# papuSpartan/stable-diffusion-webui-distributed

Hardware: NVIDIA H100
Metric: images/sec SD1.5 512x512 txt2img (higher is better)
Workload: dtype fp16

## Files before the change

stable-diffusion-webui-distributed_b200/b200sd/csrc/gemm_conv_tc.cu:

```cuda
#include <math.h>
#include <stddef.h>
#include <stdlib.h>
#include "tc_common.cuh"
#include "wgmma.cuh"
#include "b200sd_internal.h"
#include "pdl.cuh"

namespace b200sd {

constexpr int kBlockM = 128;
constexpr int kBlockK = 64;
constexpr int kMmaK = 16;
constexpr int kConsumerThreads = 256;
constexpr int kGemmThreads = kConsumerThreads + 128;
constexpr int kMaxStages = 8;
constexpr int kChunkCols = 32;
constexpr uint32_t kStageTileBytes = kBlockM * kChunkCols * 2;
constexpr uint32_t kATileBytes = kBlockM * kBlockK * 2;

struct GemmKernelParams {
  int M, N, K;
  int block_n;
  int num_m_tiles, num_n_tiles, num_k_blocks, num_stages;
  uint32_t a_bytes, b_bytes, d_bytes;
  int mode;
  int H, W, NB;
  int bw, bh, bn;
  int tiles_x, tiles_y;
  int taps, cblocks, stride, pad;
  const float* bias;
  int bias_group_rows;
  int has_residual;
  int flags;
  float res_scale;
};

struct __align__(8) GemmBarriers {
  uint64_t full[kMaxStages];
  uint64_t empty[kMaxStages];
  uint64_t res_full[2];
};

__device__ __forceinline__ float rcp_approx(float x) {
  float y;
  asm("rcp.approx.ftz.f32 %0, %1;" : "=f"(y) : "f"(x));
  return y;
}
__device__ __forceinline__ float gelu_erf(float x) {
  const float z = __fmul_rn(fabsf(x), 0.70710678118654752440f);
  float q = __fmaf_rn(0.0000430638f, z, 0.0002765672f);
  q = __fmaf_rn(q, z, 0.0001520143f);
  q = __fmaf_rn(q, z, 0.0092705272f);
  q = __fmaf_rn(q, z, 0.0422820123f);
  q = __fmaf_rn(q, z, 0.0705230784f);
  q = __fmaf_rn(q, z, 1.0f);
  q = __fmul_rn(q, q);
  q = __fmul_rn(q, q);
  q = __fmul_rn(q, q);
  q = __fmul_rn(q, q);
  const float h = __fmaf_rn(0.5f, copysignf(1.0f - rcp_approx(q), x), 0.5f);
  return __fmul_rn(x, h);
}

template <bool kBf16>
__device__ __forceinline__ uint32_t pack2(float a, float b) {
  if constexpr (kBf16) {
    __nv_bfloat162 v = __floats2bfloat162_rn(a, b);
    return *reinterpret_cast<uint32_t*>(&v);
  } else {
    __half2 v = __floats2half2_rn(a, b);
    return *reinterpret_cast<uint32_t*>(&v);
  }
}
template <bool kBf16>
__device__ __forceinline__ float2 unpack2(uint32_t u) {
  if constexpr (kBf16) {
    return __bfloat1622float2(*reinterpret_cast<__nv_bfloat162*>(&u));
  } else {
    return __half22float2(*reinterpret_cast<__half2*>(&u));
  }
}

__device__ __forceinline__ void consumer_bar_sync() {
  asm volatile("bar.sync 1, %0;" ::"n"(kConsumerThreads) : "memory");
}

struct TileCoord {
  int c1, c2, c3;
};

__device__ __forceinline__ TileCoord tile_coord(const GemmKernelParams& p, int m_tile) {
  TileCoord t;
  if (p.mode == 0) {
    t.c1 = m_tile * kBlockM; t.c2 = 0; t.c3 = 0;
  } else {
    t.c1 = (m_tile % p.tiles_x) * p.bw;
    t.c2 = ((m_tile / p.tiles_x) % p.tiles_y) * p.bh;
    t.c3 = (m_tile / (p.tiles_x * p.tiles_y)) * p.bn;
  }
  return t;
}

__device__ __forceinline__ long long tile_row(const GemmKernelParams& p, const TileCoord& tc, int m_tile, int r) {
  if (p.mode == 0) {
    const long long row = static_cast<long long>(m_tile) * kBlockM + r;
    return row < p.M ? row : 0;
  }
  const int x = tc.c1 + r % p.bw, y = tc.c2 + (r / p.bw) % p.bh, n = tc.c3 + r / (p.bw * p.bh);
  return (x < p.W && y < p.H && n < p.NB && r < p.bw * p.bh * p.bn) ? (static_cast<long long>(n) * p.H + y) * p.W + x : 0;
}

__device__ __forceinline__ void load_residual(const GemmKernelParams& p, const CUtensorMap* tmR, GemmBarriers* bars,
                                              uint8_t* stage_r, const TileCoord& tc, int n_tile, int out_bn, int c) {
  const int buf = c & 1;
  mbar_arrive_expect_tx(&bars->res_full[buf], p.d_bytes);
  const int col = n_tile * out_bn + c * kChunkCols;
  uint8_t* dst = stage_r + buf * kStageTileBytes;
  if (p.mode == 0) tma_load_2d(dst, tmR, &bars->res_full[buf], col, tc.c1);
  else tma_load_4d(dst, tmR, &bars->res_full[buf], col, tc.c1, tc.c2, tc.c3);
}

template <int BN, bool kBf16, bool kScaled>
__device__ __forceinline__ void gemm_conv_tc_body(const CUtensorMap& tmA, const CUtensorMap& tmB,
                                                  const CUtensorMap& tmD, const CUtensorMap& tmR,
                                                  const GemmKernelParams p) {
  constexpr uint32_t kStageBytes = kATileBytes + BN * 128u;
  extern __shared__ uint8_t smem_raw[];
  uint8_t* smem = reinterpret_cast<uint8_t*>((reinterpret_cast<uintptr_t>(smem_raw) + 1023) & ~uintptr_t(1023));
  uint8_t* stage_d = smem + static_cast<size_t>(p.num_stages) * kStageBytes;
  uint8_t* stage_r = stage_d + 2 * kStageTileBytes;
  GemmBarriers* bars = reinterpret_cast<GemmBarriers*>(stage_r + (p.has_residual ? 2 * kStageTileBytes : 0));

  pdl_trigger();
  const int warp = threadIdx.x >> 5;
  const int lane = threadIdx.x & 31;
  const int num_items = p.num_m_tiles * p.num_n_tiles;

  if (threadIdx.x == kConsumerThreads) {
    tma_prefetch_desc(&tmA);
    tma_prefetch_desc(&tmB);
    tma_prefetch_desc(&tmD);
    if (p.has_residual) tma_prefetch_desc(&tmR);
    for (int s = 0; s < p.num_stages; ++s) {
      mbar_init(&bars->full[s], 1);
      mbar_init(&bars->empty[s], kConsumerThreads / 128);
    }
    mbar_init(&bars->res_full[0], 1);
    mbar_init(&bars->res_full[1], 1);
    fence_mbar_init();
  }
  __syncthreads();
  pdl_wait();

  if (warp >= kConsumerThreads / 32) {
    producer_warpgroup_regs();
    if (threadIdx.x == kConsumerThreads) {
      const int nkb = p.num_k_blocks, nstages = p.num_stages, cblocks = p.cblocks;
      const bool conv = p.mode == 1, taps9 = p.taps == 9;
      const uint32_t tx_bytes = p.a_bytes + p.b_bytes;
      int stage = 0;
      uint32_t phase = 0;
      for (int item = blockIdx.x; item < num_items; item += gridDim.x) {
        const int n_tile = item % p.num_n_tiles;
        const int m_tile = item / p.num_n_tiles;
        int cx = 0, cy = 0, cn = 0;
        if (conv) {
          const int tx = m_tile % p.tiles_x;
          const int ty = (m_tile / p.tiles_x) % p.tiles_y;
          cn = (m_tile / (p.tiles_x * p.tiles_y)) * p.bn;
          cx = tx * p.bw * p.stride - p.pad;
          cy = ty * p.bh * p.stride - p.pad;
        }
        const int b_row = n_tile * BN;
        const int a_row = m_tile * kBlockM;
        int cb = 0, dx = 0, dy = 0;
        for (int kb = 0; kb < nkb; ++kb) {
          mbar_wait(&bars->empty[stage], phase ^ 1u);
          uint8_t* sA = smem + static_cast<size_t>(stage) * kStageBytes;
          uint8_t* sB = sA + kATileBytes;
          uint64_t* full_bar = &bars->full[stage];
          mbar_arrive_expect_tx(full_bar, tx_bytes);
          if (!conv) tma_load_2d(sA, &tmA, full_bar, kb * kBlockK, a_row);
          else tma_load_4d(sA, &tmA, full_bar, cb * kBlockK, cx + dx, cy + dy, cn);
          tma_load_2d(sB, &tmB, full_bar, kb * kBlockK, b_row);
          if (++cb == cblocks) {
            cb = 0;
            if (taps9 && ++dx == 3) { dx = 0; ++dy; }
          }
          if (++stage == nstages) { stage = 0; phase ^= 1u; }
        }
      }
    }
    return;
  }

  consumer_warpgroup_regs();
  const int wg = warp >> 2;
  const int row0 = wg * 64 + (warp & 3) * 16 + (lane >> 2);
  const int colq = (lane & 3) * 2;
  const bool signaller = (threadIdx.x & 127) == 0;
  const bool leader = threadIdx.x == 0;
  const bool geglu = (p.flags & B200SD_EPI_GEGLU) != 0;
  const int out_bn = geglu ? BN / 2 : BN;
  const int nchunks = out_bn / kChunkCols;
  const uint32_t smem0 = smem_u32(smem);
  float acc[BN / 2];
  int stage = 0;
  uint32_t phase = 0;
  uint32_t res_uses[2] = {0u, 0u};
  uint32_t d_slot = 0;

  for (int item = blockIdx.x; item < num_items; item += gridDim.x) {
    const int n_tile = item % p.num_n_tiles;
    const int m_tile = item / p.num_n_tiles;
    const TileCoord tc = tile_coord(p, m_tile);
    if (p.has_residual && leader) {
      load_residual(p, &tmR, bars, stage_r, tc, n_tile, out_bn, 0);
      if (nchunks > 1) load_residual(p, &tmR, bars, stage_r, tc, n_tile, out_bn, 1);
    }

    int prev_stage = 0;
    for (int kb = 0; kb < p.num_k_blocks; ++kb) {
      mbar_wait(&bars->full[stage], phase);
      const uint32_t a_addr = smem0 + static_cast<uint32_t>(stage) * kStageBytes + static_cast<uint32_t>(wg) * 8192u;
      const uint32_t b_addr = smem0 + static_cast<uint32_t>(stage) * kStageBytes + kATileBytes;
      reg_fence(acc);
      wgmma_fence();
#pragma unroll
      for (int k = 0; k < kBlockK / kMmaK; ++k)
        Wgmma<BN, kBf16>::ss(acc, make_gdesc_sw128(a_addr + 32u * k, 16, 1024), make_gdesc_sw128(b_addr + 32u * k, 16, 1024),
                             (kb | k) != 0 ? 1u : 0u);
      wgmma_commit();
      reg_fence(acc);
      wgmma_wait<1>();
      if (kb > 0 && signaller) mbar_arrive(&bars->empty[prev_stage]);
      prev_stage = stage;
      if (++stage == p.num_stages) { stage = 0; phase ^= 1u; }
    }
    wgmma_wait<0>();
    reg_fence(acc);
    if (signaller) mbar_arrive(&bars->empty[prev_stage]);

    const float* bias_r[2] = {p.bias, p.bias};
    if (p.bias != nullptr && p.bias_group_rows > 0) {
#pragma unroll
      for (int h = 0; h < 2; ++h) bias_r[h] = p.bias + (tile_row(p, tc, m_tile, row0 + 8 * h) / p.bias_group_rows) * p.N;
    }
#pragma unroll
    for (int c = 0; c < BN / kChunkCols; ++c) {
      if (c < nchunks) {
        float f[2][4][2];
#pragma unroll
        for (int g = 0; g < 4; ++g) {
          const int col = n_tile * BN + c * kChunkCols + g * 8 + colq;
#pragma unroll
          for (int h = 0; h < 2; ++h) {
            float2 b = make_float2(0.f, 0.f), bg = make_float2(0.f, 0.f);
            if (p.bias != nullptr) {
              b = __ldg(reinterpret_cast<const float2*>(bias_r[h] + col));
              if (geglu) bg = __ldg(reinterpret_cast<const float2*>(bias_r[h] + col + BN / 2));
            }
#pragma unroll
            for (int e = 0; e < 2; ++e) {
              const int idx = 4 * (4 * c + g) + 2 * h + e;
              float v = acc[idx] + (e ? b.y : b.x);
              if (geglu) {
                constexpr int kGate = BN / 4;
                v *= gelu_erf(acc[(idx + kGate) % (BN / 2)] + (e ? bg.y : bg.x));
              }
              if constexpr (kScaled) {
                if (p.flags & B200SD_EPI_LRELU) v = v > 0.f ? v : v * 0.2f;
              }
              f[h][g][e] = v;
            }
          }
        }
        if (p.has_residual) {
          const int buf = c & 1;
          mbar_wait(&bars->res_full[buf], res_uses[buf] & 1u);
          res_uses[buf]++;
          const uint8_t* rt = stage_r + buf * kStageTileBytes;
#pragma unroll
          for (int h = 0; h < 2; ++h)
#pragma unroll
            for (int g = 0; g < 4; ++g) {
              const float2 t = unpack2<kBf16>(*reinterpret_cast<const uint32_t*>(rt + sw64_offset(row0 + 8 * h, g) + colq * 2));
              if constexpr (kScaled) {
                f[h][g][0] = __fmaf_rn(p.res_scale, f[h][g][0], t.x);
                f[h][g][1] = __fmaf_rn(p.res_scale, f[h][g][1], t.y);
              } else {
                f[h][g][0] += t.x;
                f[h][g][1] += t.y;
              }
            }
        }
        if (!kScaled && (p.flags & B200SD_EPI_SILU)) {
#pragma unroll
          for (int h = 0; h < 2; ++h)
#pragma unroll
            for (int g = 0; g < 4; ++g)
#pragma unroll
              for (int e = 0; e < 2; ++e) f[h][g][e] = __fdividef(f[h][g][e], 1.0f + __expf(-f[h][g][e]));
        }
        uint8_t* dt = stage_d + d_slot * kStageTileBytes;
#pragma unroll
        for (int h = 0; h < 2; ++h)
#pragma unroll
          for (int g = 0; g < 4; ++g)
            *reinterpret_cast<uint32_t*>(dt + sw64_offset(row0 + 8 * h, g) + colq * 2) = pack2<kBf16>(f[h][g][0], f[h][g][1]);
        fence_proxy_async_smem();
        if (leader) bulk_wait_read<0>();
        consumer_bar_sync();
        if (leader) {
          const int col = n_tile * out_bn + c * kChunkCols;
          if (p.mode == 0) tma_store_2d(&tmD, dt, col, tc.c1);
          else tma_store_4d(&tmD, dt, col, tc.c1, tc.c2, tc.c3);
          bulk_commit();
          if (p.has_residual && c + 2 < nchunks) load_residual(p, &tmR, bars, stage_r, tc, n_tile, out_bn, c + 2);
        }
        d_slot ^= 1u;
      }
    }
  }
  if (leader) bulk_wait<0>();
}

template <int BN, bool kBf16>
__global__ void __launch_bounds__(kGemmThreads, 1)
gemm_conv_tc_kernel(const __grid_constant__ CUtensorMap tmA, const __grid_constant__ CUtensorMap tmB,
                    const __grid_constant__ CUtensorMap tmD, const __grid_constant__ CUtensorMap tmR,
                    const GemmKernelParams p) {
  gemm_conv_tc_body<BN, kBf16, false>(tmA, tmB, tmD, tmR, p);
}

template <int BN, bool kBf16>
__global__ void __launch_bounds__(kGemmThreads, 1)
conv_scaled_tc_kernel(const __grid_constant__ CUtensorMap tmA, const __grid_constant__ CUtensorMap tmB,
                      const __grid_constant__ CUtensorMap tmD, const __grid_constant__ CUtensorMap tmR,
                      const GemmKernelParams p) {
  gemm_conv_tc_body<BN, kBf16, true>(tmA, tmB, tmD, tmR, p);
}

typedef void (*GemmKernel)(CUtensorMap, CUtensorMap, CUtensorMap, CUtensorMap, GemmKernelParams);

static GemmKernel scaled_kernel_for(int block_n, int is_bf16) {
  if (is_bf16) return nullptr;
  if (block_n == 32) return conv_scaled_tc_kernel<32, false>;
  if (block_n == 64) return conv_scaled_tc_kernel<64, false>;
  return nullptr;
}

template <bool kBf16>
static GemmKernel kernel_for(int block_n) {
  switch (block_n) {
    case 32: return gemm_conv_tc_kernel<32, kBf16>;
    case 64: return gemm_conv_tc_kernel<64, kBf16>;
    case 96: return gemm_conv_tc_kernel<96, kBf16>;
    case 128: return gemm_conv_tc_kernel<128, kBf16>;
    case 160: return gemm_conv_tc_kernel<160, kBf16>;
    case 192: return gemm_conv_tc_kernel<192, kBf16>;
    case 224: return gemm_conv_tc_kernel<224, kBf16>;
    case 256: return gemm_conv_tc_kernel<256, kBf16>;
    default: return nullptr;
  }
}
static GemmKernel kernel_for(int block_n, int is_bf16) {
  return is_bf16 ? kernel_for<true>(block_n) : kernel_for<false>(block_n);
}

static int g_num_sms = 0;
static int g_max_smem = 0;
static bool g_dev_ready[64] = {};
static int device_props() {
  int dev = 0;
  if (cudaGetDevice(&dev) != cudaSuccess) return B200SD_ERR_CUDA;
  if (dev < 0 || dev >= 64) return B200SD_ERR_UNSUPPORTED;
  if (!g_dev_ready[dev]) {
    int sms = 0, smem = 0;
    if (cudaDeviceGetAttribute(&sms, cudaDevAttrMultiProcessorCount, dev) != cudaSuccess) return B200SD_ERR_CUDA;
    if (cudaDeviceGetAttribute(&smem, cudaDevAttrMaxSharedMemoryPerBlockOptin, dev) != cudaSuccess)
      return B200SD_ERR_CUDA;
    for (int bn = 32; bn <= 256; bn += 32)
      for (int bf = 0; bf < 2; ++bf)
        for (GemmKernel k : {kernel_for(bn, bf), scaled_kernel_for(bn, bf)})
          if (k != nullptr && cudaFuncSetAttribute(k, cudaFuncAttributeMaxDynamicSharedMemorySize, smem) != cudaSuccess)
            return B200SD_ERR_CUDA;
    g_num_sms = sms;
    g_max_smem = smem;
    g_dev_ready[dev] = true;
  }
  return B200SD_OK;
}

static int launch(const CUtensorMap& tmA, const CUtensorMap& tmB, const CUtensorMap& tmD, const CUtensorMap& tmR,
                  GemmKernelParams& p, int is_bf16, int max_ctas, cudaStream_t stream, bool scaled = false) {
  const uint32_t stage_bytes = kATileBytes + static_cast<uint32_t>(p.block_n) * 128u;
  const int staging = (p.has_residual ? 4 : 2) * static_cast<int>(kStageTileBytes);
  const int budget = g_max_smem - 1024  - staging - static_cast<int>(sizeof(GemmBarriers));
  int stages = budget / static_cast<int>(stage_bytes);
  if (stages > kMaxStages) stages = kMaxStages;
  if (stages < 2) return B200SD_ERR_UNSUPPORTED;
  p.num_stages = stages;
  const size_t smem = 1024 + static_cast<size_t>(stages) * stage_bytes + staging + sizeof(GemmBarriers);
  const int num_tiles = p.num_m_tiles * p.num_n_tiles;
  int grid = num_tiles < g_num_sms ? num_tiles : g_num_sms;
  if (max_ctas > 0 && grid > max_ctas) grid = max_ctas;
  if (grid <= 0) return B200SD_OK;
  GemmKernel k = scaled ? scaled_kernel_for(p.block_n, is_bf16) : kernel_for(p.block_n, is_bf16);
  if (k == nullptr) return B200SD_ERR_INVALID;
  launch_pdl(k, dim3(grid), dim3(kGemmThreads), smem, stream, tmA, tmB, tmD, tmR, p);
  return cudaGetLastError() == cudaSuccess ? B200SD_OK : B200SD_ERR_CUDA;
}

struct OutSpec {
  void* D;
  long long ldd;
  const void* residual;
  long long ldr;
  int n_out;
};

static int fill_common(GemmKernelParams& p, OutSpec& o, int M, int N, int K, int block_n, const b200sd_epilogue* epi,
                       void* D, long long ldd, int is_bf16) {
  if (block_n < 32 || block_n > 256 || block_n % 32 != 0 || N % block_n != 0 || K % kBlockK != 0) return B200SD_ERR_INVALID;
  p.M = M; p.N = N; p.K = K; p.block_n = block_n;
  p.num_n_tiles = N / block_n;
  p.num_k_blocks = K / kBlockK;
  p.b_bytes = static_cast<uint32_t>(block_n) * 128u;
  p.bias = epi ? epi->bias : nullptr;
  p.bias_group_rows = epi ? epi->bias_group_rows : 0;
  p.flags = epi ? epi->flags : 0;
  o.D = D; o.ldd = ldd;
  o.residual = epi ? epi->residual : nullptr;
  o.ldr = epi ? epi->ldr : 0;
  p.has_residual = o.residual != nullptr ? 1 : 0;
  const bool geglu = (p.flags & B200SD_EPI_GEGLU) != 0;
  if (geglu && block_n % 64 != 0) return B200SD_ERR_INVALID;
  o.n_out = geglu ? N / 2 : N;
  if (ldd % 8 != 0 || (reinterpret_cast<uintptr_t>(D) & 15) != 0) return B200SD_ERR_INVALID;
  if (o.residual && (o.ldr % 8 != 0 || (reinterpret_cast<uintptr_t>(o.residual) & 15) != 0)) return B200SD_ERR_INVALID;
  if (p.bias && (reinterpret_cast<uintptr_t>(p.bias) & 15) != 0) return B200SD_ERR_INVALID;
  return B200SD_OK;
}

static int make_out_maps(const GemmKernelParams& p, const OutSpec& o, CUtensorMap* tmD, CUtensorMap* tmR) {
  int rc;
  for (int which = 0; which < 2; ++which) {
    const void* base = which == 0 ? o.D : o.residual;
    const long long ld = which == 0 ? o.ldd : o.ldr;
    CUtensorMap* out = which == 0 ? tmD : tmR;
    if (base == nullptr) {
      *tmR = *tmD;
      continue;
    }
    if (p.mode == 0) {
      const uint64_t dims[2] = {static_cast<uint64_t>(o.n_out), static_cast<uint64_t>(p.M)};
      const uint64_t strides[1] = {static_cast<uint64_t>(ld) * 2};
      const uint32_t box[2] = {kChunkCols, kBlockM};
      const uint32_t es[2] = {1, 1};
      rc = make_tmap_sw64(out, base, 2, dims, strides, box, es);
    } else {
      const uint64_t dims[4] = {static_cast<uint64_t>(o.n_out), static_cast<uint64_t>(p.W), static_cast<uint64_t>(p.H),
                                static_cast<uint64_t>(p.NB)};
      const uint64_t strides[3] = {static_cast<uint64_t>(ld) * 2, static_cast<uint64_t>(ld) * 2 * p.W,
                                   static_cast<uint64_t>(ld) * 2 * p.W * p.H};
      const uint32_t box[4] = {kChunkCols, static_cast<uint32_t>(p.bw), static_cast<uint32_t>(p.bh),
                               static_cast<uint32_t>(p.bn)};
      const uint32_t es[4] = {1, 1, 1, 1};
      rc = make_tmap_sw64(out, base, 4, dims, strides, box, es);
    }
    if (rc != B200SD_OK) return rc;
  }
  return B200SD_OK;
}

int gemm_tc(const void* A, long long lda, const void* Wt, void* D, long long ldd, int M, int N, int K, int block_n,
            const b200sd_epilogue* epi, int is_bf16, int max_ctas, cudaStream_t stream) {
  if (M <= 0) return B200SD_OK;
  GemmKernelParams p{};
  OutSpec o{};
  int rc = fill_common(p, o, M, N, K, block_n, epi, D, ldd, is_bf16);
  if (rc != B200SD_OK) return rc;
  if (lda % 8 != 0 || (reinterpret_cast<uintptr_t>(A) & 15) != 0 || (reinterpret_cast<uintptr_t>(Wt) & 15) != 0)
    return B200SD_ERR_INVALID;
  p.mode = 0;
  p.num_m_tiles = (M + kBlockM - 1) / kBlockM;
  p.a_bytes = 16384u;
  p.d_bytes = kStageTileBytes;
  rc = device_props();
  if (rc != B200SD_OK) return rc;
  CUtensorMap tmA, tmB, tmD, tmR;
  {
    const uint64_t dims[2] = {static_cast<uint64_t>(K), static_cast<uint64_t>(M)};
    const uint64_t strides[1] = {static_cast<uint64_t>(lda) * 2};
    const uint32_t box[2] = {kBlockK, kBlockM};
    const uint32_t es[2] = {1, 1};
    rc = make_tmap_sw128(&tmA, A, 2, dims, strides, box, es);
    if (rc != B200SD_OK) return rc;
  }
  {
    const uint64_t dims[2] = {static_cast<uint64_t>(K), static_cast<uint64_t>(N)};
    const uint64_t strides[1] = {static_cast<uint64_t>(K) * 2};
    const uint32_t box[2] = {kBlockK, static_cast<uint32_t>(block_n)};
    const uint32_t es[2] = {1, 1};
    rc = make_tmap_sw128(&tmB, Wt, 2, dims, strides, box, es);
    if (rc != B200SD_OK) return rc;
  }
  rc = make_out_maps(p, o, &tmD, &tmR);
  if (rc != B200SD_OK) return rc;
  return launch(tmA, tmB, tmD, tmR, p, is_bf16, max_ctas, stream);
}

int conv_tc(const void* X, long long pitch_c, int NB, int Hin, int Win, int C, const void* Wt, int ksize, int stride,
            int pad, int pad_end, void* D, long long ldd, int Cout, int block_n, const b200sd_epilogue* epi,
            int is_bf16, int max_ctas, cudaStream_t stream, bool scaled, float res_scale) {
  if (NB <= 0) return B200SD_OK;
  if ((ksize != 3 && ksize != 1) || (stride != 1 && stride != 2) || C % kBlockK != 0) return B200SD_ERR_INVALID;
  if (scaled && epi != nullptr && (epi->flags & ~B200SD_EPI_LRELU) != 0) return B200SD_ERR_INVALID;
  if (pitch_c % 8 != 0 || (reinterpret_cast<uintptr_t>(X) & 15) != 0 || (reinterpret_cast<uintptr_t>(Wt) & 15) != 0)
    return B200SD_ERR_INVALID;
  const int taps = ksize * ksize;
  const int Ho = (Hin + pad + pad_end - ksize) / stride + 1;
  const int Wo = (Win + pad + pad_end - ksize) / stride + 1;
  if (Ho <= 0 || Wo <= 0) return B200SD_ERR_INVALID;
  GemmKernelParams p{};
  OutSpec o{};
  int rc = fill_common(p, o, NB * Ho * Wo, Cout, taps * C, block_n, epi, D, ldd, is_bf16);
  if (rc != B200SD_OK) return rc;
  p.mode = 1;
  p.res_scale = res_scale;
  p.H = Ho; p.W = Wo; p.NB = NB;
  p.taps = taps; p.cblocks = C / kBlockK; p.stride = stride; p.pad = pad;
  p.bw = Wo < kBlockM ? Wo : kBlockM;
  p.bh = kBlockM / p.bw; if (p.bh > Ho) p.bh = Ho; if (p.bh < 1) p.bh = 1;
  p.bn = kBlockM / (p.bw * p.bh); if (p.bn > NB) p.bn = NB; if (p.bn < 1) p.bn = 1;
  p.tiles_x = (Wo + p.bw - 1) / p.bw;
  p.tiles_y = (Ho + p.bh - 1) / p.bh;
  const int tiles_n = (NB + p.bn - 1) / p.bn;
  p.num_m_tiles = p.tiles_x * p.tiles_y * tiles_n;
  p.a_bytes = static_cast<uint32_t>(p.bw * p.bh * p.bn) * 128u;
  p.d_bytes = static_cast<uint32_t>(p.bw * p.bh * p.bn) * kChunkCols * 2u;
  rc = device_props();
  if (rc != B200SD_OK) return rc;
  CUtensorMap tmA, tmB, tmD, tmR;
  {
    const uint64_t dims[4] = {static_cast<uint64_t>(C), static_cast<uint64_t>(Win), static_cast<uint64_t>(Hin),
                              static_cast<uint64_t>(NB)};
    const uint64_t strides[3] = {static_cast<uint64_t>(pitch_c) * 2, static_cast<uint64_t>(pitch_c) * 2 * Win,
                                 static_cast<uint64_t>(pitch_c) * 2 * Win * Hin};
    const uint32_t box[4] = {kBlockK, static_cast<uint32_t>(p.bw * stride), static_cast<uint32_t>(p.bh * stride),
                             static_cast<uint32_t>(p.bn)};
    const uint32_t es[4] = {1, static_cast<uint32_t>(stride), static_cast<uint32_t>(stride), 1};
    if (box[1] > 256 || box[2] > 256) return B200SD_ERR_UNSUPPORTED;
    rc = make_tmap_sw128(&tmA, X, 4, dims, strides, box, es);
    if (rc != B200SD_OK) return rc;
  }
  {
    const uint64_t K = static_cast<uint64_t>(taps) * C;
    const uint64_t dims[2] = {K, static_cast<uint64_t>(Cout)};
    const uint64_t strides[1] = {K * 2};
    const uint32_t box[2] = {kBlockK, static_cast<uint32_t>(block_n)};
    const uint32_t es[2] = {1, 1};
    rc = make_tmap_sw128(&tmB, Wt, 2, dims, strides, box, es);
    if (rc != B200SD_OK) return rc;
  }
  rc = make_out_maps(p, o, &tmD, &tmR);
  if (rc != B200SD_OK) return rc;
  return launch(tmA, tmB, tmD, tmR, p, is_bf16, max_ctas, stream, scaled);
}

}
```

stable-diffusion-webui-distributed_b200/b200sd/ops.py:

```python
import ctypes
from typing import Optional

import torch

from . import _lib
from ._lib import BF16, EPI_GEGLU, EPI_LRELU, EPI_SILU, F16, Epilogue, check

LAUNCHES = 0


def _count(n: int = 1):
    global LAUNCHES
    LAUNCHES += n


def _dt(t: torch.Tensor) -> int:
    if t.dtype == torch.float16:
        return F16
    if t.dtype == torch.bfloat16:
        return BF16
    raise TypeError(f"b200sd ops take fp16/bf16 activations, got {t.dtype}")


def _stream() -> ctypes.c_void_p:
    return ctypes.c_void_p(torch.cuda.current_stream().cuda_stream)


def _p(t: Optional[torch.Tensor]) -> ctypes.c_void_p:
    return ctypes.c_void_p(0 if t is None else t.data_ptr())


def _rows2d(t: torch.Tensor):
    assert t.stride(-1) == 1, "last dim must be contiguous"
    cols = t.shape[-1]
    pitch = t.stride(-2) if t.dim() >= 2 else cols
    rows = t.numel() // cols
    exp = pitch
    for d in range(t.dim() - 2, -1, -1):
        if t.shape[d] != 1:
            assert t.stride(d) == exp, f"tensor is not row-collapsible: shape {tuple(t.shape)} stride {t.stride()}"
        exp *= t.shape[d]
    return rows, cols, pitch


def _epi(bias, bias_group_rows, residual, flags):
    e = Epilogue()
    e.bias = 0 if bias is None else bias.data_ptr()
    e.bias_group_rows = int(bias_group_rows)
    e.residual = 0 if residual is None else residual.data_ptr()
    e.ldr = 0 if residual is None else _rows2d(residual)[2]
    e.flags = int(flags)
    if bias is not None:
        assert bias.dtype == torch.float32 and bias.is_contiguous()
    return e


NUM_SMS = 132


def pick_block_n(n: int, geglu: bool = False, m: Optional[int] = None) -> int:
    cands = [bn for bn in (160, 128, 96, 64, 32) if n % bn == 0 and (not geglu or bn % 64 == 0)]
    if not cands:
        raise ValueError(f"N={n} has no supported tile width")
    if geglu or m is None:
        return cands[0]
    mt = (m + 127) // 128
    best = None
    for bn in cands:
        if bn < 128 <= cands[0]:
            continue
        tiles = mt * (n // bn)
        waves = -(-tiles // NUM_SMS)
        score = tiles / (waves * NUM_SMS) * (1.0 if bn >= 160 else 0.97 if bn >= 128 else 0.93)
        if best is None or score > best[0] + 1e-9:
            best = (score, bn)
    return best[1]


def linear(a: torch.Tensor, wt: torch.Tensor, out: torch.Tensor, bias: Optional[torch.Tensor] = None,
           bias_group_rows: int = 0, residual: Optional[torch.Tensor] = None, flags: int = 0,
           block_n: Optional[int] = None, max_ctas: int = 0):
    m, k, lda = _rows2d(a)
    n, k2 = wt.shape
    assert k == k2 and wt.is_contiguous()
    mo, no, ldd = _rows2d(out)
    geglu = bool(flags & EPI_GEGLU)
    assert mo == m and no == (n // 2 if geglu else n), (mo, m, no, n)
    bn = block_n or pick_block_n(n, geglu, m)
    e = _epi(bias, bias_group_rows, residual, flags)
    rc = _lib.lib().b200sd_linear(_p(a), ctypes.c_longlong(lda), _p(wt), _p(out), ctypes.c_longlong(ldd), m, n, k, bn,
                                  ctypes.byref(e), _dt(a), max_ctas, _stream())
    check(rc, f"b200sd_linear M={m} N={n} K={k} bn={bn}")
    _count()
    return out


def conv2d(x: torch.Tensor, wt: torch.Tensor, out: torch.Tensor, ksize: int, stride: int = 1, pad: int = 1,
           pad_end: Optional[int] = None, bias: Optional[torch.Tensor] = None, bias_group_rows: int = 0,
           residual: Optional[torch.Tensor] = None, flags: int = 0, block_n: Optional[int] = None, max_ctas: int = 0):
    nb, h, w, c = x.shape
    assert x.stride(3) == 1 and x.stride(1) == w * x.stride(2) and x.stride(0) == h * x.stride(1)
    cout, kk = wt.shape
    assert kk == ksize * ksize * c and wt.is_contiguous()
    pe = pad if pad_end is None else pad_end
    mo, no, ldd = _rows2d(out)
    bn = block_n or pick_block_n(cout, False, mo)
    e = _epi(bias, bias_group_rows, residual, flags)
    rc = _lib.lib().b200sd_conv2d(_p(x), ctypes.c_longlong(x.stride(2)), nb, h, w, c, _p(wt), ksize, stride, pad, pe,
                                  _p(out), ctypes.c_longlong(ldd), cout, bn, ctypes.byref(e), _dt(x), max_ctas,
                                  _stream())
    check(rc, f"b200sd_conv2d NB={nb} H={h} W={w} C={c} Cout={cout} k={ksize} s={stride}")
    _count()
    return out


def attention(q: torch.Tensor, k: torch.Tensor, v: torch.Tensor, out: torch.Tensor, heads: int, d: int, d_pad: int,
              scale: float, v_ones_col: bool = False, kv_len: Optional[torch.Tensor] = None):
    b, sq, _ = q.shape
    skv = k.shape[1]
    for t in (q, k, v, out):
        assert t.stride(2) == 1 and t.stride(0) == t.shape[1] * t.stride(1)
    if kv_len is None:
        rc = _lib.lib().b200sd_attention(_p(q), ctypes.c_longlong(q.stride(1)), _p(k), ctypes.c_longlong(k.stride(1)),
                                         _p(v), ctypes.c_longlong(v.stride(1)), _p(out), ctypes.c_longlong(out.stride(1)),
                                         b, heads, sq, skv, d, d_pad, ctypes.c_float(scale), int(bool(v_ones_col)),
                                         _dt(q), _stream())
        check(rc, f"b200sd_attention B={b} h={heads} Sq={sq} Skv={skv} d={d}")
    else:
        assert kv_len.dtype == torch.int32 and kv_len.is_contiguous() and kv_len.numel() == b
        assert kv_len.device == q.device, "kv_len must live on the device"
        rc = _lib.lib().b200sd_attention_varlen(_p(q), ctypes.c_longlong(q.stride(1)), _p(k),
                                                ctypes.c_longlong(k.stride(1)), _p(v), ctypes.c_longlong(v.stride(1)),
                                                _p(out), ctypes.c_longlong(out.stride(1)), b, heads, sq, skv,
                                                _p(kv_len), d, d_pad, ctypes.c_float(scale), int(bool(v_ones_col)),
                                                _dt(q), _stream())
        check(rc, f"b200sd_attention_varlen B={b} h={heads} Sq={sq} Skv={skv} d={d}")
    _count()
    return out


_GN_FLOATS = {}


def groupnorm_stats_floats(nb: int, hw: int, c: int, groups: int) -> int:
    key = (nb, hw, c, groups)
    n = _GN_FLOATS.get(key)
    if n is None:
        n = int(_lib.lib().b200sd_groupnorm_stats_floats(nb, hw, c, groups))
        if n < 0:
            raise _lib.B200SDError(f"groupnorm: unsupported shape C={c}")
        _GN_FLOATS[key] = n
    return n


def groupnorm(x: torch.Tensor, out: torch.Tensor, stats: torch.Tensor, gamma: torch.Tensor, beta: torch.Tensor,
              groups: int, eps: float, silu: bool):
    nb, hw, c = x.shape
    assert x.stride(2) == 1 and out.stride(2) == 1 and x.stride(0) == hw * x.stride(1)
    assert stats.dtype == torch.float32 and stats.is_contiguous()
    assert stats.numel() >= groupnorm_stats_floats(nb, hw, c, groups), "stats buffer too small"
    rc = _lib.lib().b200sd_groupnorm(_p(x), ctypes.c_longlong(x.stride(1)), _p(out), ctypes.c_longlong(out.stride(1)), nb,
                                     hw, c, groups, _p(stats), _p(gamma), _p(beta), ctypes.c_float(eps), int(silu),
                                     _dt(x), _stream())
    check(rc, "b200sd_groupnorm")
    _count(2)
    return out


def layernorm(x: torch.Tensor, out: torch.Tensor, gamma: torch.Tensor, beta: torch.Tensor, eps: float = 1e-5):
    rows, c, ldx = _rows2d(x)
    _, _, ldy = _rows2d(out)
    rc = _lib.lib().b200sd_layernorm(_p(x), ctypes.c_longlong(ldx), _p(out), ctypes.c_longlong(ldy), rows, c, _p(gamma),
                                     _p(beta), ctypes.c_float(eps), _dt(x), _stream())
    check(rc, "b200sd_layernorm")
    _count()
    return out


def upsample2x(x: torch.Tensor, out: torch.Tensor):
    nb, h, w, c = x.shape
    rc = _lib.lib().b200sd_upsample2x(_p(x), ctypes.c_longlong(x.stride(2)), _p(out), ctypes.c_longlong(out.stride(2)),
                                      nb, h, w, c, _dt(x), _stream())
    check(rc, "b200sd_upsample2x")
    _count()
    return out


def pad_circular(x: torch.Tensor, out: torch.Tensor, p: int):
    nb, h, w, c = x.shape
    for t in (x, out):
        assert t.stride(3) == 1 and t.stride(1) == t.shape[2] * t.stride(2) and t.stride(0) == t.shape[1] * t.stride(1)
    assert out.shape == (nb, h + 2 * p, w + 2 * p, c) and out.dtype == x.dtype, (tuple(x.shape), tuple(out.shape), p)
    rc = _lib.lib().b200sd_pad_circular(_p(x), ctypes.c_longlong(x.stride(2)), _p(out), ctypes.c_longlong(out.stride(2)),
                                        nb, h, w, c, p, _dt(x), _stream())
    check(rc, f"b200sd_pad_circular NB={nb} H={h} W={w} C={c} p={p}")
    _count()
    return out


def softmax_rows_(s: torch.Tensor, scale: float):
    rows, cols, lds = _rows2d(s)
    rc = _lib.lib().b200sd_softmax_rows(_p(s), ctypes.c_longlong(lds), rows, cols, ctypes.c_float(scale), _dt(s),
                                        _stream())
    check(rc, "b200sd_softmax_rows")
    _count()
    return s


def silu(x: torch.Tensor, out: torch.Tensor):
    assert x.is_contiguous() and out.is_contiguous()
    rc = _lib.lib().b200sd_silu(_p(x), _p(out), ctypes.c_longlong(x.numel()), _dt(x), _stream())
    check(rc, "b200sd_silu")
    _count()
    return out


def timestep_embedding(t: torch.Tensor, out: torch.Tensor):
    assert t.dtype == torch.float32 and t.is_contiguous()
    rc = _lib.lib().b200sd_timestep_embedding(_p(t), t.numel(), out.shape[1], _p(out), ctypes.c_longlong(out.stride(0)),
                                              _dt(out), _stream())
    check(rc, "b200sd_timestep_embedding")
    _count()
    return out


def fold_bias(emb: torch.Tensor, bias: torch.Tensor, table: torch.Tensor):
    t, c = table.shape
    assert table.dtype == torch.float32 and table.is_contiguous() and bias.numel() == c
    rc = _lib.lib().b200sd_fold_bias(_p(emb), ctypes.c_longlong(emb.stride(0)), _p(bias), _p(table), t, c, _dt(emb),
                                     _stream())
    check(rc, "b200sd_fold_bias")
    _count()
    return table


def select_step(table: torch.Tensor, step_counter: torch.Tensor, cur: torch.Tensor):
    assert table.dtype == torch.float32 and cur.dtype == torch.float32 and step_counter.dtype == torch.int32
    rc = _lib.lib().b200sd_select_step(_p(table), ctypes.c_longlong(table.shape[1]), _p(step_counter), _p(cur), _stream())
    check(rc, "b200sd_select_step")
    _count()
    return cur


def select_context(bank: torch.Tensor, entry_len: torch.Tensor, sched: torch.Tensor, step_counter: torch.Tensor,
                   ctx: torch.Tensor, kv_len: torch.Tensor):
    e, cap, c = bank.shape
    rows = ctx.shape[0]
    assert tuple(ctx.shape) == (rows, cap, c) and ctx.dtype == bank.dtype and bank.is_contiguous() and ctx.is_contiguous()
    assert sched.dim() == 2 and sched.shape[1] == rows and sched.is_contiguous() and entry_len.numel() >= e
    assert all(t.dtype == torch.int32 for t in (entry_len, sched, step_counter, kv_len)) and kv_len.numel() == rows
    _dt(ctx)
    rc = _lib.lib().b200sd_select_context(_p(bank), _p(entry_len), e, _p(sched), _p(step_counter), _p(ctx), _p(kv_len),
                                          rows, cap, c, _stream())
    check(rc, "b200sd_select_context")
    _count()
    return ctx


def pack_unet_input(x: torch.Tensor, xin: torch.Tensor, in_scale: float = 1.0):
    b, hw, _ = x.shape
    rc = _lib.lib().b200sd_pack_unet_input(_p(x), _p(xin), ctypes.c_longlong(xin.stride(1)), b, hw,
                                           ctypes.c_float(in_scale), _dt(xin), _stream())
    check(rc, "b200sd_pack_unet_input")
    _count()
    return xin


def cfg_ddim_step(eps: torch.Tensor, x: torch.Tensor, xin: torch.Tensor, cfg_scale: float, coef: torch.Tensor,
                  step_counter: torch.Tensor):
    b, hw, _ = x.shape
    rc = _lib.lib().b200sd_cfg_ddim_step(_p(eps), ctypes.c_longlong(eps.stride(1)), _p(x), _p(xin),
                                         ctypes.c_longlong(xin.stride(1)), b, hw, ctypes.c_float(cfg_scale), _p(coef),
                                         _p(step_counter), _dt(xin), _stream())
    check(rc, "b200sd_cfg_ddim_step")
    _count(2)


def cfg_euler_a_step(eps: torch.Tensor, x: torch.Tensor, noise: Optional[torch.Tensor], xin: torch.Tensor,
                     cfg_scale: float, coef: torch.Tensor, step_counter: torch.Tensor):
    b, hw, _ = x.shape
    rc = _lib.lib().b200sd_cfg_euler_a_step(_p(eps), ctypes.c_longlong(eps.stride(1)), _p(x), _p(noise), _p(xin),
                                            ctypes.c_longlong(xin.stride(1)), b, hw, ctypes.c_float(cfg_scale),
                                            _p(coef), _p(step_counter), _dt(xin), _stream())
    check(rc, "b200sd_cfg_euler_a_step")
    _count(2)


def cfg_dpmpp_2m_step(eps: torch.Tensor, x: torch.Tensor, old_denoised: torch.Tensor, xin: torch.Tensor,
                      cfg_scale: float, coef8: torch.Tensor, step_counter: torch.Tensor):
    b, hw, _ = x.shape
    assert coef8.shape[-1] == 8 and old_denoised.shape == x.shape
    rc = _lib.lib().b200sd_cfg_dpmpp_2m_step(_p(eps), ctypes.c_longlong(eps.stride(1)), _p(x), _p(old_denoised), _p(xin),
                                             ctypes.c_longlong(xin.stride(1)), b, hw, ctypes.c_float(cfg_scale),
                                             _p(coef8), _p(step_counter), _dt(xin), _stream())
    check(rc, "b200sd_cfg_dpmpp_2m_step")
    _count(2)



def cfg_ddim_step_v(v: torch.Tensor, x: torch.Tensor, xin: torch.Tensor, cfg_scale: float, coef: torch.Tensor,
                    step_counter: torch.Tensor):
    b, hw, _ = x.shape
    rc = _lib.lib().b200sd_cfg_ddim_step_v(_p(v), ctypes.c_longlong(v.stride(1)), _p(x), _p(xin),
                                           ctypes.c_longlong(xin.stride(1)), b, hw, ctypes.c_float(cfg_scale), _p(coef),
                                           _p(step_counter), _dt(xin), _stream())
    check(rc, "b200sd_cfg_ddim_step_v")
    _count(2)


def cfg_euler_a_step_v(v: torch.Tensor, x: torch.Tensor, noise: Optional[torch.Tensor], xin: torch.Tensor,
                       cfg_scale: float, coef8: torch.Tensor, step_counter: torch.Tensor):
    b, hw, _ = x.shape
    assert coef8.shape[-1] == 8
    rc = _lib.lib().b200sd_cfg_euler_a_step_v(_p(v), ctypes.c_longlong(v.stride(1)), _p(x), _p(noise), _p(xin),
                                              ctypes.c_longlong(xin.stride(1)), b, hw, ctypes.c_float(cfg_scale),
                                              _p(coef8), _p(step_counter), _dt(xin), _stream())
    check(rc, "b200sd_cfg_euler_a_step_v")
    _count(2)


def cfg_dpmpp_2m_step_v(v: torch.Tensor, x: torch.Tensor, old_denoised: torch.Tensor, xin: torch.Tensor,
                        cfg_scale: float, coef8: torch.Tensor, step_counter: torch.Tensor):
    b, hw, _ = x.shape
    assert coef8.shape[-1] == 8 and old_denoised.shape == x.shape
    rc = _lib.lib().b200sd_cfg_dpmpp_2m_step_v(_p(v), ctypes.c_longlong(v.stride(1)), _p(x), _p(old_denoised), _p(xin),
                                               ctypes.c_longlong(xin.stride(1)), b, hw, ctypes.c_float(cfg_scale),
                                               _p(coef8), _p(step_counter), _dt(xin), _stream())
    check(rc, "b200sd_cfg_dpmpp_2m_step_v")
    _count(2)

def image_to_nhwc(img_u8: torch.Tensor, out: torch.Tensor):
    b, hw, _ = img_u8.shape
    assert img_u8.dtype == torch.uint8 and img_u8.is_contiguous()
    rc = _lib.lib().b200sd_image_to_nhwc(_p(img_u8), _p(out), ctypes.c_longlong(out.stride(1)), b, hw, _dt(out), _stream())
    check(rc, "b200sd_image_to_nhwc")
    _count()
    return out


def hint_to_nhwc(img_u8: torch.Tensor, out: torch.Tensor):
    b, hw, _ = img_u8.shape
    assert img_u8.dtype == torch.uint8 and img_u8.is_contiguous()
    assert out.shape[:2] == (b, hw) and out.stride(2) == 1 and out.stride(0) == hw * out.stride(1)
    rc = _lib.lib().b200sd_hint_to_nhwc(_p(img_u8), _p(out), ctypes.c_longlong(out.stride(1)), b, hw, _dt(out), _stream())
    check(rc, "b200sd_hint_to_nhwc")
    _count()
    return out


def masked_image_to_nhwc(img_u8: torch.Tensor, mask_u8: Optional[torch.Tensor], weight: float, out: torch.Tensor):
    b, hw, _ = img_u8.shape
    assert img_u8.dtype == torch.uint8 and img_u8.is_contiguous()
    assert out.shape[:2] == (b, hw) and out.stride(2) == 1 and out.stride(0) == hw * out.stride(1)
    assert mask_u8 is None or (mask_u8.dtype == torch.uint8 and mask_u8.is_contiguous() and mask_u8.numel() == hw)
    rc = _lib.lib().b200sd_masked_image_to_nhwc(_p(img_u8), _p(mask_u8), ctypes.c_float(weight), _p(out),
                                                ctypes.c_longlong(out.stride(1)), b, hw, _dt(out), _stream())
    check(rc, "b200sd_masked_image_to_nhwc")
    _count()
    return out


def pack_image_cond(z: torch.Tensor, mask_u8: Optional[torch.Tensor], xin: torch.Tensor, h: int, w: int):
    b = z.shape[0]
    assert z.dtype == torch.float32 and z.is_contiguous() and z.shape == (b, h * w, 4)
    assert xin.shape[:2] == (2 * b, h * w) and xin.stride(2) == 1 and xin.stride(0) == h * w * xin.stride(1)
    f = 1
    if mask_u8 is not None:
        f = mask_u8.shape[0] // h
        assert mask_u8.dtype == torch.uint8 and mask_u8.is_contiguous() and tuple(mask_u8.shape) == (f * h, f * w), \
            (tuple(mask_u8.shape), h, w)
    rc = _lib.lib().b200sd_pack_image_cond(_p(z), _p(mask_u8), _p(xin), ctypes.c_longlong(xin.stride(1)), b, h, w, f,
                                           _dt(xin), _stream())
    check(rc, "b200sd_pack_image_cond")
    _count()
    return xin


def unpack_latent(moments: torch.Tensor, x: torch.Tensor, scale: float):
    b, hw, _ = moments.shape
    assert x.dtype == torch.float32 and x.is_contiguous()
    rc = _lib.lib().b200sd_unpack_latent(_p(moments), ctypes.c_longlong(moments.stride(1)), _p(x), b, hw,
                                         ctypes.c_float(scale), _dt(moments), _stream())
    check(rc, "b200sd_unpack_latent")
    _count()
    return x


def quantize_u8(img: torch.Tensor, out: torch.Tensor):
    b, hw, _ = img.shape
    assert out.dtype == torch.uint8 and out.is_contiguous()
    rc = _lib.lib().b200sd_quantize_u8(_p(img), ctypes.c_longlong(img.stride(1)), _p(out), b, hw, _dt(img), _stream())
    check(rc, "b200sd_quantize_u8")
    _count()
    return out


def blend_latent(x: torch.Tensor, init: torch.Tensor, latmask: torch.Tensor):
    b, hw, _ = x.shape
    assert x.dtype == init.dtype == latmask.dtype == torch.float32 and x.is_contiguous() and init.is_contiguous()
    assert init.shape == x.shape and latmask.shape == (hw,) and latmask.is_contiguous()
    rc = _lib.lib().b200sd_blend_latent(_p(x), _p(init), _p(latmask), b, hw, _stream())
    check(rc, "b200sd_blend_latent")
    _count()
    return x


def resize_latent_bilinear(x: torch.Tensor, y: torch.Tensor, h: int, w: int, ho: int, wo: int):
    b = x.shape[0]
    assert x.dtype == torch.float32 and y.dtype == torch.float32 and x.is_contiguous() and y.is_contiguous()
# ... 173 lines not shown
```

Baseline: 12.30.

## Ping-pong consumer warpgroups for narrow tiles and producer-driven residual loads

```diff
diff --git a/stable-diffusion-webui-distributed_b200/b200sd/csrc/gemm_conv_tc.cu b/stable-diffusion-webui-distributed_b200/b200sd/csrc/gemm_conv_tc.cu
--- a/stable-diffusion-webui-distributed_b200/b200sd/csrc/gemm_conv_tc.cu
+++ b/stable-diffusion-webui-distributed_b200/b200sd/csrc/gemm_conv_tc.cu
@@ -35,10 +35,13 @@
   float res_scale;
 };
 
+__host__ __device__ constexpr int consumer_groups(int block_n) { return block_n <= 128 ? 2 : 1; }
+
 struct __align__(8) GemmBarriers {
   uint64_t full[kMaxStages];
   uint64_t empty[kMaxStages];
   uint64_t res_full[2];
+  uint64_t res_empty[2];
 };
 
 __device__ __forceinline__ float rcp_approx(float x) {
@@ -81,8 +84,14 @@
   }
 }
 
-__device__ __forceinline__ void consumer_bar_sync() {
-  asm volatile("bar.sync 1, %0;" ::"n"(kConsumerThreads) : "memory");
+__device__ __forceinline__ void group_bar_sync(int group, int threads) {
+  asm volatile("bar.sync %0, %1;" ::"r"(4 + group), "r"(threads) : "memory");
+}
+__device__ __forceinline__ void turn_wait(int group) {
+  asm volatile("bar.sync %0, 256;" ::"r"(2 + group) : "memory");
+}
+__device__ __forceinline__ void turn_pass(int group) {
+  asm volatile("bar.arrive %0, 256;" ::"r"(3 - group) : "memory");
 }
 
 struct TileCoord {
@@ -110,14 +119,15 @@
   return (x < p.W && y < p.H && n < p.NB && r < p.bw * p.bh * p.bn) ? (static_cast<long long>(n) * p.H + y) * p.W + x : 0;
 }
 
-__device__ __forceinline__ void load_residual(const GemmKernelParams& p, const CUtensorMap* tmR, GemmBarriers* bars,
-                                              uint8_t* stage_r, const TileCoord& tc, int n_tile, int out_bn, int c) {
-  const int buf = c & 1;
-  mbar_arrive_expect_tx(&bars->res_full[buf], p.d_bytes);
-  const int col = n_tile * out_bn + c * kChunkCols;
-  uint8_t* dst = stage_r + buf * kStageTileBytes;
-  if (p.mode == 0) tma_load_2d(dst, tmR, &bars->res_full[buf], col, tc.c1);
-  else tma_load_4d(dst, tmR, &bars->res_full[buf], col, tc.c1, tc.c2, tc.c3);
+__device__ __forceinline__ void load_residual(const GemmKernelParams& p, const CUtensorMap* tmR, uint64_t* bar,
+                                              uint8_t* dst, const TileCoord& tc, int n_tile, int out_bn, int nchunks) {
+  mbar_arrive_expect_tx(bar, static_cast<uint32_t>(nchunks) * p.d_bytes);
+  for (int c = 0; c < nchunks; ++c) {
+    const int col = n_tile * out_bn + c * kChunkCols;
+    uint8_t* d = dst + c * kStageTileBytes;
+    if (p.mode == 0) tma_load_2d(d, tmR, bar, col, tc.c1);
+    else tma_load_4d(d, tmR, bar, col, tc.c1, tc.c2, tc.c3);
+  }
 }
 
 template <int BN, bool kBf16, bool kScaled>
@@ -125,16 +135,23 @@
                                                   const CUtensorMap& tmD, const CUtensorMap& tmR,
                                                   const GemmKernelParams p) {
   constexpr uint32_t kStageBytes = kATileBytes + BN * 128u;
+  constexpr int kGroups = consumer_groups(BN);
+  constexpr int kWgPerTile = 2 / kGroups;
+  constexpr int kHalves = kGroups;
   extern __shared__ uint8_t smem_raw[];
   uint8_t* smem = reinterpret_cast<uint8_t*>((reinterpret_cast<uintptr_t>(smem_raw) + 1023) & ~uintptr_t(1023));
-  uint8_t* stage_d = smem + static_cast<size_t>(p.num_stages) * kStageBytes;
-  uint8_t* stage_r = stage_d + 2 * kStageTileBytes;
-  GemmBarriers* bars = reinterpret_cast<GemmBarriers*>(stage_r + (p.has_residual ? 2 * kStageTileBytes : 0));
+  const bool geglu = (p.flags & B200SD_EPI_GEGLU) != 0;
+  const int out_bn = geglu ? BN / 2 : BN;
+  const int nchunks = out_bn / kChunkCols;
+  const uint32_t out_tile_bytes = static_cast<uint32_t>(nchunks) * kStageTileBytes;
+  uint8_t* stage_e = smem + static_cast<size_t>(p.num_stages) * kStageBytes;
+  GemmBarriers* bars = reinterpret_cast<GemmBarriers*>(stage_e + kGroups * out_tile_bytes);
 
   pdl_trigger();
   const int warp = threadIdx.x >> 5;
   const int lane = threadIdx.x & 31;
   const int num_items = p.num_m_tiles * p.num_n_tiles;
+  const int ntiles = (num_items - static_cast<int>(blockIdx.x) + static_cast<int>(gridDim.x) - 1) / static_cast<int>(gridDim.x);
 
   if (threadIdx.x == kConsumerThreads) {
     tma_prefetch_desc(&tmA);
@@ -143,10 +160,12 @@
     if (p.has_residual) tma_prefetch_desc(&tmR);
     for (int s = 0; s < p.num_stages; ++s) {
       mbar_init(&bars->full[s], 1);
-      mbar_init(&bars->empty[s], kConsumerThreads / 128);
-    }
-    mbar_init(&bars->res_full[0], 1);
-    mbar_init(&bars->res_full[1], 1);
+      mbar_init(&bars->empty[s], kWgPerTile);
+    }
+    for (int g = 0; g < 2; ++g) {
+      mbar_init(&bars->res_full[g], 1);
+      mbar_init(&bars->res_empty[g], 1);
+    }
     fence_mbar_init();
   }
   __syncthreads();
@@ -160,7 +179,8 @@
       const uint32_t tx_bytes = p.a_bytes + p.b_bytes;
       int stage = 0;
       uint32_t phase = 0;
-      for (int item = blockIdx.x; item < num_items; item += gridDim.x) {
+      for (int i = 0; i < ntiles; ++i) {
+        const int item = blockIdx.x + i * gridDim.x;
         const int n_tile = item % p.num_n_tiles;
         const int m_tile = item / p.num_n_tiles;
         int cx = 0, cy = 0, cn = 0;
@@ -189,6 +209,12 @@
           }
           if (++stage == nstages) { stage = 0; phase ^= 1u; }
         }
+        if (p.has_residual) {
+          const int g = i % kGroups;
+          mbar_wait(&bars->res_empty[g], ((i / kGroups) & 1) ^ 1u);
+          load_residual(p, &tmR, &bars->res_full[g], stage_e + g * out_tile_bytes, tile_coord(p, m_tile), n_tile, out_bn,
+                        nchunks);
+        }
       }
     }
     return;
@@ -196,130 +222,137 @@
 
   consumer_warpgroup_regs();
   const int wg = warp >> 2;
-  const int row0 = wg * 64 + (warp & 3) * 16 + (lane >> 2);
+  const int group = kGroups == 2 ? wg : 0;
+  const int wg_row = kGroups == 2 ? 0 : wg * 64;
+  const int row0 = wg_row + (warp & 3) * 16 + (lane >> 2);
   const int colq = (lane & 3) * 2;
   const bool signaller = (threadIdx.x & 127) == 0;
-  const bool leader = threadIdx.x == 0;
-  const bool geglu = (p.flags & B200SD_EPI_GEGLU) != 0;
-  const int out_bn = geglu ? BN / 2 : BN;
-  const int nchunks = out_bn / kChunkCols;
+  const bool leader = (threadIdx.x & (128 * kWgPerTile - 1)) == 0;
   const uint32_t smem0 = smem_u32(smem);
-  float acc[BN / 2];
-  int stage = 0;
-  uint32_t phase = 0;
-  uint32_t res_uses[2] = {0u, 0u};
-  uint32_t d_slot = 0;
-
-  for (int item = blockIdx.x; item < num_items; item += gridDim.x) {
+  uint8_t* out_tile = stage_e + group * out_tile_bytes;
+  float acc[kHalves][BN / 2];
+
+  if (kGroups == 2 && group == 1) turn_pass(1);
+  for (int i = group; i < ntiles; i += kGroups) {
+    const int item = blockIdx.x + i * gridDim.x;
     const int n_tile = item % p.num_n_tiles;
     const int m_tile = item / p.num_n_tiles;
     const TileCoord tc = tile_coord(p, m_tile);
-    if (p.has_residual && leader) {
-      load_residual(p, &tmR, bars, stage_r, tc, n_tile, out_bn, 0);
-      if (nchunks > 1) load_residual(p, &tmR, bars, stage_r, tc, n_tile, out_bn, 1);
-    }
-
+    const int ring = i * p.num_k_blocks;
+    int stage = ring % p.num_stages;
+    uint32_t phase = static_cast<uint32_t>(ring / p.num_stages) & 1u;
+
+    if (kGroups == 2) turn_wait(group);
     int prev_stage = 0;
     for (int kb = 0; kb < p.num_k_blocks; ++kb) {
-      mbar_wait(&bars->full[stage], phase);
-      const uint32_t a_addr = smem0 + static_cast<uint32_t>(stage) * kStageBytes + static_cast<uint32_t>(wg) * 8192u;
+      mbar_wait_unbounded(&bars->full[stage], phase);
+      const uint32_t a_addr = smem0 + static_cast<uint32_t>(stage) * kStageBytes + static_cast<uint32_t>(wg_row) * 128u;
       const uint32_t b_addr = smem0 + static_cast<uint32_t>(stage) * kStageBytes + kATileBytes;
-      reg_fence(acc);
+#pragma unroll
+      for (int hh = 0; hh < kHalves; ++hh) reg_fence(acc[hh]);
       wgmma_fence();
 #pragma unroll
       for (int k = 0; k < kBlockK / kMmaK; ++k)
-        Wgmma<BN, kBf16>::ss(acc, make_gdesc_sw128(a_addr + 32u * k, 16, 1024), make_gdesc_sw128(b_addr + 32u * k, 16, 1024),
-                             (kb | k) != 0 ? 1u : 0u);
+#pragma unroll
+        for (int hh = 0; hh < kHalves; ++hh)
+          Wgmma<BN, kBf16>::ss(acc[hh], make_gdesc_sw128(a_addr + 8192u * hh + 32u * k, 16, 1024),
+                               make_gdesc_sw128(b_addr + 32u * k, 16, 1024), (kb | k) != 0 ? 1u : 0u);
       wgmma_commit();
-      reg_fence(acc);
+#pragma unroll
+      for (int hh = 0; hh < kHalves; ++hh) reg_fence(acc[hh]);
       wgmma_wait<1>();
       if (kb > 0 && signaller) mbar_arrive(&bars->empty[prev_stage]);
       prev_stage = stage;
       if (++stage == p.num_stages) { stage = 0; phase ^= 1u; }
     }
+    if (kGroups == 2 && i + 1 < ntiles) turn_pass(group);
     wgmma_wait<0>();
-    reg_fence(acc);
+#pragma unroll
+    for (int hh = 0; hh < kHalves; ++hh) reg_fence(acc[hh]);
     if (signaller) mbar_arrive(&bars->empty[prev_stage]);
 
-    const float* bias_r[2] = {p.bias, p.bias};
-    if (p.bias != nullptr && p.bias_group_rows > 0) {
-#pragma unroll
-      for (int h = 0; h < 2; ++h) bias_r[h] = p.bias + (tile_row(p, tc, m_tile, row0 + 8 * h) / p.bias_group_rows) * p.N;
-    }
+    if (p.has_residual) mbar_wait_unbounded(&bars->res_full[group], static_cast<uint32_t>(i / kGroups) & 1u);
+    else group_bar_sync(group, 128 * kWgPerTile);
 #pragma unroll
     for (int c = 0; c < BN / kChunkCols; ++c) {
       if (c < nchunks) {
-        float f[2][4][2];
-#pragma unroll
-        for (int g = 0; g < 4; ++g) {
-          const int col = n_tile * BN + c * kChunkCols + g * 8 + colq;
-#pragma unroll
-          for (int h = 0; h < 2; ++h) {
-            float2 b = make_float2(0.f, 0.f), bg = make_float2(0.f, 0.f);
-            if (p.bias != nullptr) {
-              b = __ldg(reinterpret_cast<const float2*>(bias_r[h] + col));
-              if (geglu) bg = __ldg(reinterpret_cast<const float2*>(bias_r[h] + col + BN / 2));
-            }
-#pragma unroll
-            for (int e = 0; e < 2; ++e) {
-              const int idx = 4 * (4 * c + g) + 2 * h + e;
-              float v = acc[idx] + (e ? b.y : b.x);
-              if (geglu) {
-                constexpr int kGate = BN / 4;
-                v *= gelu_erf(acc[(idx + kGate) % (BN / 2)] + (e ? bg.y : bg.x));
+        uint8_t* dt = out_tile + c * kStageTileBytes;
+#pragma unroll
+        for (int hh = 0; hh < kHalves; ++hh) {
+          const int r = row0 + 64 * hh;
+          const float* bias_r[2] = {p.bias, p.bias};
+          if (p.bias != nullptr && p.bias_group_rows > 0) {
+#pragma unroll
+            for (int h = 0; h < 2; ++h) bias_r[h] = p.bias + (tile_row(p, tc, m_tile, r + 8 * h) / p.bias_group_rows) * p.N;
+          }
+          float f[2][4][2];
+#pragma unroll
+          for (int g = 0; g < 4; ++g) {
+            const int col = n_tile * BN + c * kChunkCols + g * 8 + colq;
+#pragma unroll
+            for (int h = 0; h < 2; ++h) {
+              float2 b = make_float2(0.f, 0.f), bg = make_float2(0.f, 0.f);
+              if (p.bias != nullptr) {
+                b = __ldg(reinterpret_cast<const float2*>(bias_r[h] + col));
+                if (geglu) bg = __ldg(reinterpret_cast<const float2*>(bias_r[h] + col + BN / 2));
               }
-              if constexpr (kScaled) {
-                if (p.flags & B200SD_EPI_LRELU) v = v > 0.f ? v : v * 0.2f;
+#pragma unroll
+              for (int e = 0; e < 2; ++e) {
+                const int idx = 4 * (4 * c + g) + 2 * h + e;
+                float v = acc[hh][idx] + (e ? b.y : b.x);
+                if (geglu) {
+                  constexpr int kGate = BN / 4;
+                  v *= gelu_erf(acc[hh][(idx + kGate) % (BN / 2)] + (e ? bg.y : bg.x));
+                }
+                if constexpr (kScaled) {
+                  if (p.flags & B200SD_EPI_LRELU) v = v > 0.f ? v : v * 0.2f;
+                }
+                f[h][g][e] = v;
               }
-              f[h][g][e] = v;
             }
           }
+          if (p.has_residual) {
+#pragma unroll
+            for (int h = 0; h < 2; ++h)
+#pragma unroll
+              for (int g = 0; g < 4; ++g) {
+                const float2 t = unpack2<kBf16>(*reinterpret_cast<const uint32_t*>(dt + sw64_offset(r + 8 * h, g) + colq * 2));
+                if constexpr (kScaled) {
+                  f[h][g][0] = __fmaf_rn(p.res_scale, f[h][g][0], t.x);
+                  f[h][g][1] = __fmaf_rn(p.res_scale, f[h][g][1], t.y);
+                } else {
+                  f[h][g][0] += t.x;
+                  f[h][g][1] += t.y;
+                }
+              }
+          }
+          if (!kScaled && (p.flags & B200SD_EPI_SILU)) {
+#pragma unroll
+            for (int h = 0; h < 2; ++h)
+#pragma unroll
+              for (int g = 0; g < 4; ++g)
+#pragma unroll
+                for (int e = 0; e < 2; ++e) f[h][g][e] = __fdividef(f[h][g][e], 1.0f + __expf(-f[h][g][e]));
+          }
+#pragma unroll
+          for (int h = 0; h < 2; ++h)
+#pragma unroll
+            for (int g = 0; g < 4; ++g)
+              *reinterpret_cast<uint32_t*>(dt + sw64_offset(r + 8 * h, g) + colq * 2) = pack2<kBf16>(f[h][g][0], f[h][g][1]);
         }
-        if (p.has_residual) {
-          const int buf = c & 1;
-          mbar_wait(&bars->res_full[buf], res_uses[buf] & 1u);
-          res_uses[buf]++;
-          const uint8_t* rt = stage_r + buf * kStageTileBytes;
-#pragma unroll
-          for (int h = 0; h < 2; ++h)
-#pragma unroll
-            for (int g = 0; g < 4; ++g) {
-              const float2 t = unpack2<kBf16>(*reinterpret_cast<const uint32_t*>(rt + sw64_offset(row0 + 8 * h, g) + colq * 2));
-              if constexpr (kScaled) {
-                f[h][g][0] = __fmaf_rn(p.res_scale, f[h][g][0], t.x);
-                f[h][g][1] = __fmaf_rn(p.res_scale, f[h][g][1], t.y);
-              } else {
-                f[h][g][0] += t.x;
-                f[h][g][1] += t.y;
-              }
-            }
-        }
-        if (!kScaled && (p.flags & B200SD_EPI_SILU)) {
-#pragma unroll
-          for (int h = 0; h < 2; ++h)
-#pragma unroll
-            for (int g = 0; g < 4; ++g)
-#pragma unroll
-              for (int e = 0; e < 2; ++e) f[h][g][e] = __fdividef(f[h][g][e], 1.0f + __expf(-f[h][g][e]));
-        }
-        uint8_t* dt = stage_d + d_slot * kStageTileBytes;
-#pragma unroll
-        for (int h = 0; h < 2; ++h)
-#pragma unroll
-          for (int g = 0; g < 4; ++g)
-            *reinterpret_cast<uint32_t*>(dt + sw64_offset(row0 + 8 * h, g) + colq * 2) = pack2<kBf16>(f[h][g][0], f[h][g][1]);
         fence_proxy_async_smem();
-        if (leader) bulk_wait_read<0>();
-        consumer_bar_sync();
+        group_bar_sync(group, 128 * kWgPerTile);
         if (leader) {
           const int col = n_tile * out_bn + c * kChunkCols;
           if (p.mode == 0) tma_store_2d(&tmD, dt, col, tc.c1);
           else tma_store_4d(&tmD, dt, col, tc.c1, tc.c2, tc.c3);
           bulk_commit();
-          if (p.has_residual && c + 2 < nchunks) load_residual(p, &tmR, bars, stage_r, tc, n_tile, out_bn, c + 2);
         }
-        d_slot ^= 1u;
       }
+    }
+    if (leader) {
+      bulk_wait_read<0>();
+      if (p.has_residual) mbar_arrive(&bars->res_empty[group]);
     }
   }
   if (leader) bulk_wait<0>();
@@ -395,7 +428,8 @@
 static int launch(const CUtensorMap& tmA, const CUtensorMap& tmB, const CUtensorMap& tmD, const CUtensorMap& tmR,
                   GemmKernelParams& p, int is_bf16, int max_ctas, cudaStream_t stream, bool scaled = false) {
   const uint32_t stage_bytes = kATileBytes + static_cast<uint32_t>(p.block_n) * 128u;
-  const int staging = (p.has_residual ? 4 : 2) * static_cast<int>(kStageTileBytes);
+  const int out_bn = (p.flags & B200SD_EPI_GEGLU) ? p.block_n / 2 : p.block_n;
+  const int staging = consumer_groups(p.block_n) * (out_bn / kChunkCols) * static_cast<int>(kStageTileBytes);
   const int budget = g_max_smem - 1024  - staging - static_cast<int>(sizeof(GemmBarriers));
   int stages = budget / static_cast<int>(stage_bytes);
   if (stages > kMaxStages) stages = kMaxStages;
diff --git a/stable-diffusion-webui-distributed_b200/b200sd/ops.py b/stable-diffusion-webui-distributed_b200/b200sd/ops.py
--- a/stable-diffusion-webui-distributed_b200/b200sd/ops.py
+++ b/stable-diffusion-webui-distributed_b200/b200sd/ops.py
@@ -58,8 +58,10 @@
 NUM_SMS = 132
 
 
-def pick_block_n(n: int, geglu: bool = False, m: Optional[int] = None) -> int:
-    cands = [bn for bn in (160, 128, 96, 64, 32) if n % bn == 0 and (not geglu or bn % 64 == 0)]
+def pick_block_n(n: int, geglu: bool = False, m: Optional[int] = None, k: Optional[int] = None) -> int:
+    wide = m is not None and k is not None and m * k >= (1 << 28) and not geglu and n % 1280 == 0
+    cands = [bn for bn in ((256,) if wide else ()) + (160, 128, 96, 64, 32)
+             if n % bn == 0 and (not geglu or bn % 64 == 0)]
     if not cands:
         raise ValueError(f"N={n} has no supported tile width")
     if geglu or m is None:
@@ -71,7 +73,7 @@
             continue
         tiles = mt * (n // bn)
         waves = -(-tiles // NUM_SMS)
-        score = tiles / (waves * NUM_SMS) * (1.0 if bn >= 160 else 0.97 if bn >= 128 else 0.93)
+        score = tiles / (waves * NUM_SMS) * (1.02 if bn == 256 else 1.0 if bn >= 160 else 0.97 if bn >= 128 else 0.93)
         if best is None or score > best[0] + 1e-9:
             best = (score, bn)
     return best[1]
@@ -86,7 +88,7 @@
     mo, no, ldd = _rows2d(out)
     geglu = bool(flags & EPI_GEGLU)
     assert mo == m and no == (n // 2 if geglu else n), (mo, m, no, n)
-    bn = block_n or pick_block_n(n, geglu, m)
+    bn = block_n or pick_block_n(n, geglu, m, k)
     e = _epi(bias, bias_group_rows, residual, flags)
     rc = _lib.lib().b200sd_linear(_p(a), ctypes.c_longlong(lda), _p(wt), _p(out), ctypes.c_longlong(ldd), m, n, k, bn,
                                   ctypes.byref(e), _dt(a), max_ctas, _stream())
@@ -104,7 +106,7 @@
     assert kk == ksize * ksize * c and wt.is_contiguous()
     pe = pad if pad_end is None else pad_end
     mo, no, ldd = _rows2d(out)
-    bn = block_n or pick_block_n(cout, False, mo)
+    bn = block_n or pick_block_n(cout, False, mo, kk)
     e = _epi(bias, bias_group_rows, residual, flags)
     rc = _lib.lib().b200sd_conv2d(_p(x), ctypes.c_longlong(x.stride(2)), nb, h, w, c, _p(wt), ksize, stride, pad, pe,
                                   _p(out), ctypes.c_longlong(ldd), cout, bn, ctypes.byref(e), _dt(x), max_ctas,
```

Result: no change. 12.42 (median of 6 runs) (+1.0%).
